# deu439/ARFlow

Hardware: AMD Instinct MI355X
Metric: image-pairs/sec fwd+bwd, PWCLite 384x640 bs=8 (higher is better)
Workload: dtype f32; 1 GPU; pwclite_uflow+uflow_loss, 384x640 pairs, batch 8 per GPU, fwd(both directions)+loss+bwd+allreduce+Adam; global_batch=8, parallelism=dp1, step_start=seeded weights + fresh Adam state, restored before every step, loss_finite=True

## Files before the change

### arflow_amd/_lib.py

```python
import ctypes
import os

_HERE = os.path.dirname(os.path.abspath(__file__))
LIB_PATH = os.path.join(_HERE, 'csrc', 'libarflow_hip.so')

c_fp = ctypes.c_void_p
c_i = ctypes.c_int
c_l = ctypes.c_long
c_f = ctypes.c_float

PROTOTYPES = {
    'arflow_abi_version': [],
    'arflow_take_stale_error': [],
    'arflow_set_deterministic': [c_i],
    'arflow_get_deterministic': [],
    'arflow_flow_up_fwd': [c_fp, c_fp, c_i, c_i, c_i, c_i, c_i, c_fp],
    'arflow_flow_up_bwd': [c_fp, c_fp, c_i, c_i, c_i, c_i, c_i, c_fp],
    'arflow_out_up2_fwd': [c_fp, c_l, c_fp, c_l, c_i, c_i, c_i, c_i, c_i, c_i, c_f, c_fp],
    'arflow_out_up2_bwd': [c_fp, c_l, c_fp, c_l, c_i, c_i, c_i, c_i, c_i, c_fp],
    'arflow_out_tail_fwd': [c_fp, c_l, c_fp, c_fp, c_i, c_i, c_i, c_i, c_i, c_i, c_f, c_fp],
    'arflow_prob_up_fwd': [c_fp, c_l, c_fp, c_l, c_i, c_i, c_i, c_i, c_i, c_i, c_i, c_f, c_fp],
    'arflow_prob_up_bwd': [c_fp, c_l, c_fp, c_l, c_i, c_i, c_i, c_i, c_i, c_i, c_fp],
    'arflow_profile_marker': [c_i, c_fp],
    'arflow_sums_rows': [c_i, c_i, c_i],
    'arflow_corr_fwd': [c_fp, c_fp, c_fp, c_fp, c_i, c_i, c_i, c_i, c_i, c_f, c_fp],
    'arflow_corr_sign_planes': [c_i, c_i, c_i],
    'arflow_corr_strided_supported': [c_i, c_i, c_i],
    'arflow_corr_fwd_strided': [c_fp, c_fp, c_fp, c_l, c_fp, c_i, c_i, c_i, c_i, c_i, c_f, c_fp],
    'arflow_corr_bwd_strided': [c_fp, c_l, c_fp, c_l, c_fp, c_fp, c_fp, c_fp, c_fp, c_i, c_i, c_i, c_i, c_i, c_f, c_fp],
    'arflow_corr_bwd': [c_fp, c_fp, c_fp, c_fp, c_fp, c_fp, c_fp, c_i, c_i, c_i, c_i, c_i, c_f, c_fp],
    'arflow_corr_fwd_bf16': [c_fp, c_fp, c_fp, c_i, c_i, c_i, c_i, c_i, c_f, c_fp],
    'arflow_corr_bwd_bf16': [c_fp, c_fp, c_fp, c_fp, c_fp, c_fp, c_i, c_i, c_i, c_i, c_i, c_f, c_fp],
    'arflow_warp_fwd_bf16': [c_fp, c_fp, c_fp, c_fp, c_i, c_i, c_i, c_i, c_i, c_i, c_l, c_i, c_i, c_i, c_fp],
    'arflow_warp_bwd_bf16': [c_fp, c_fp, c_fp, c_fp, c_fp, c_i, c_i, c_i, c_i, c_i, c_i, c_l, c_i, c_i, c_i, c_fp],
    'arflow_warp_nearest_fwd': [c_fp, c_fp, c_fp, c_i, c_i, c_i, c_i, c_i, c_i, c_l, c_i, c_i, c_i, c_fp],
    'arflow_warp_nearest_bwd': [c_fp, c_fp, c_fp, c_i, c_i, c_i, c_i, c_i, c_i, c_l, c_i, c_i, c_i, c_fp],
    'arflow_warp_bicubic_fwd': [c_fp, c_fp, c_fp, c_i, c_i, c_i, c_i, c_i, c_i, c_l, c_i, c_i, c_i, c_fp],
    'arflow_warp_bicubic_bwd': [c_fp, c_fp, c_fp, c_fp, c_fp, c_i, c_i, c_i, c_i, c_i, c_i, c_l, c_i, c_i, c_i, c_fp],
    'arflow_ssim_fwd': [c_fp, c_fp, c_fp, c_i, c_i, c_i, c_i, c_i, c_fp],
    'arflow_ssim_bwd': [c_fp, c_fp, c_fp, c_fp, c_i, c_i, c_i, c_i, c_i, c_fp],
    'arflow_corr_general_out_size': [c_i, c_i, c_i, c_i, c_i, c_i, c_i, c_fp, c_fp, c_fp],
    'arflow_corr_general_fwd': [c_fp, c_fp, c_fp, c_i, c_i, c_i, c_i, c_i, c_i, c_i, c_i, c_i, c_fp],
    'arflow_corr_general_bwd': [c_fp, c_fp, c_fp, c_fp, c_fp, c_i, c_i, c_i, c_i, c_i, c_i, c_i, c_i, c_i, c_fp],
    'arflow_featnorm_fwd': [c_fp, c_fp, c_fp, c_fp, c_fp, c_fp, c_i, c_l, c_i, c_fp],
    'arflow_featnorm_bwd': [c_fp, c_fp, c_fp, c_fp, c_fp, c_fp, c_fp, c_fp, c_i, c_l, c_i, c_fp],
    'arflow_level_supported': [c_i, c_i, c_i],
    'arflow_level_bwd_ws_bytes': [c_i, c_i, c_i, c_i],
    'arflow_level_fwd': [c_fp, c_fp, c_fp, c_l, c_i, c_i, c_fp, c_fp, c_l, c_fp, c_i, c_fp, c_l, c_fp, c_l, c_fp, c_fp, c_fp, c_i, c_i, c_i, c_i, c_i, c_f, c_i, c_i, c_i, c_fp],
    'arflow_level_bwd': [c_fp, c_l, c_fp, c_fp, c_l, c_fp, c_l, c_fp, c_fp, c_fp, c_fp, c_l, c_fp, c_l, c_fp, c_fp, c_i, c_fp, c_fp, c_fp, c_i, c_i, c_fp, c_i, c_i, c_i, c_i, c_i, c_f, c_i, c_i, c_i, c_fp],
    'arflow_level_fwd_m': [c_fp, c_fp, c_fp, c_l, c_i, c_i, c_fp, c_fp, c_l, c_fp, c_i, c_fp, c_l, c_fp, c_l, c_fp, c_fp, c_fp, c_fp, c_i, c_fp, c_i, c_i, c_i, c_i, c_i, c_i, c_f, c_i, c_i, c_i, c_fp],
    'arflow_up2_bwd': [c_fp, c_fp, c_i, c_i, c_i, c_i, c_fp],
    'arflow_bias_act_mom_rows': [c_i, c_l],
    'arflow_bias_act_fwd_mom': [c_fp, c_fp, c_fp, c_fp, c_i, c_i, c_l, c_f, c_fp],
    'arflow_level_acc_rows': [c_i, c_i, c_i, c_i, c_i],
    'arflow_level_moments': [c_fp, c_fp, c_fp, c_i, c_l, c_fp],
    'arflow_level_warp_fwd': [c_fp, c_fp, c_fp, c_l, c_i, c_i, c_fp, c_fp, c_l, c_fp, c_fp, c_i, c_i, c_i, c_i, c_i, c_i, c_i, c_fp],
    'arflow_level_corr_fwd': [c_fp, c_fp, c_fp, c_i, c_i, c_fp, c_l, c_fp, c_l, c_fp, c_fp, c_i, c_i, c_i, c_i, c_i, c_f, c_fp],
    'arflow_level_corr_bwd': [c_fp, c_l, c_fp, c_fp, c_l, c_fp, c_fp, c_fp, c_fp, c_i, c_i, c_i, c_i, c_i, c_f, c_fp],
    'arflow_bias_act_fwd': [c_fp, c_fp, c_fp, c_i, c_i, c_l, c_f, c_fp],
    'arflow_bias_act_bwd': [c_fp, c_fp, c_fp, c_fp, c_i, c_i, c_l, c_f, c_fp],
    'arflow_headconv_fwd': [c_fp, c_fp, c_fp, c_fp, c_i, c_i, c_i, c_i, c_fp],
    'arflow_headconv_bwd_data': [c_fp, c_fp, c_fp, c_i, c_i, c_i, c_i, c_fp],
    'arflow_headconv_bwd_weight_ws_bytes': [c_i, c_i, c_i, c_i],
    'arflow_headconv_bwd_weight': [c_fp, c_fp, c_fp, c_fp, c_fp, c_i, c_i, c_i, c_i, c_fp],
    'arflow_splitconv_pack_bytes': [c_i, c_i],
    'arflow_splitconv_pack': [c_fp, c_fp, c_i, c_i, c_i, c_fp],
    'arflow_splitconv_fwd': [c_fp, c_fp, c_fp, c_i, c_i, c_i, c_i, c_i, c_fp],
    'arflow_dense_cat_fwd': [c_fp, c_fp, c_fp, c_fp, c_i, c_i, c_i, c_l, c_f, c_fp],
    'arflow_dense_gbias_rows': [c_i, c_l],
    'arflow_dense_grad_gather': [c_fp, c_i, c_fp, c_l, c_fp, c_fp, c_i, c_i, c_l, c_f, c_fp],
    'arflow_warp_fwd': [c_fp, c_fp, c_fp, c_fp, c_i, c_i, c_i, c_i, c_i, c_i, c_l, c_i, c_i, c_i, c_fp],
    'arflow_warp_bwd': [c_fp, c_fp, c_fp, c_fp, c_fp, c_i, c_i, c_i, c_i, c_i, c_i, c_l, c_i, c_i, c_i, c_fp],
    'arflow_splat_map': [c_fp, c_fp, c_i, c_i, c_i, c_l, c_i, c_fp],
    'arflow_coord_mask': [c_fp, c_fp, c_i, c_i, c_i, c_l, c_i, c_fp],
    'arflow_occ_bidir': [c_fp, c_fp, c_fp, c_i, c_i, c_i, c_l, c_l, c_f, c_f, c_fp],
    'arflow_census_fwd': [c_fp, c_fp, c_fp, c_fp, c_fp, c_fp, c_i, c_i, c_i, c_i, c_fp],
    'arflow_census_bwd': [c_fp, c_fp, c_fp, c_fp, c_fp, c_i, c_i, c_i, c_i, c_fp],
    'arflow_census_warp_supported': [c_i, c_i],
    'arflow_census_warp_fwd': [c_fp, c_fp, c_fp, c_l, c_fp, c_fp, c_fp, c_fp, c_i, c_i, c_i, c_i, c_fp],
    'arflow_census_warp_bwd': [c_fp, c_fp, c_fp, c_l, c_fp, c_fp, c_fp, c_i, c_i, c_i, c_i, c_fp],
    'arflow_census_warp_pair_fwd': [c_fp, c_fp, c_l, c_fp, c_fp, c_fp, c_fp, c_i, c_i, c_i, c_i, c_fp],
    'arflow_census_warp_pair_bwd': [c_fp, c_fp, c_l, c_fp, c_fp, c_fp, c_i, c_i, c_i, c_i, c_fp],
    'arflow_uflow_pair_bwd': [c_fp, c_fp, c_l, c_fp, c_fp, c_fp, c_i, c_i, c_i, c_i, c_fp, c_l, c_fp, c_fp, c_fp, c_i, c_i, c_f, c_f, c_i, c_i, c_i, c_fp],
    'arflow_down4_gray_z': [c_fp, c_fp, c_fp, c_fp, c_i, c_i, c_i, c_fp],
    'arflow_splat_smooth_fwd': [c_fp, c_fp, c_fp, c_fp, c_i, c_i, c_i, c_l, c_f, c_f, c_i, c_i, c_i, c_i, c_fp],
    'arflow_down4_gray': [c_fp, c_fp, c_fp, c_i, c_i, c_i, c_fp],
    'arflow_photo_fwd': [c_fp, c_fp, c_fp, c_fp, c_fp, c_i, c_i, c_i, c_i, c_fp],
    'arflow_photo_bwd': [c_fp, c_fp, c_fp, c_fp, c_fp, c_fp, c_i, c_i, c_i, c_i, c_fp],
    'arflow_photo_warp_rows': [c_i, c_i, c_i],
    'arflow_photo_warp_fwd': [c_fp, c_l, c_l, c_fp, c_l, c_l, c_fp, c_l, c_l, c_fp, c_l, c_l, c_i, c_i, c_i, c_i, c_fp, c_fp, c_i, c_i, c_i, c_i, c_i, c_i, c_fp],
    'arflow_photo_warp_bwd': [c_fp, c_l, c_l, c_fp, c_l, c_l, c_fp, c_l, c_l, c_fp, c_l, c_l, c_i, c_i, c_i, c_i, c_fp, c_fp, c_l, c_l, c_i, c_i, c_i, c_i, c_i, c_i, c_fp],
    'arflow_area_pyramid_ws_bytes': [c_i, c_i, c_i, c_fp, c_i],
    'arflow_area_pyramid': [c_fp, c_fp, c_i, c_i, c_i, c_fp, c_i, c_fp],
    'arflow_smooth_fwd': [c_fp, c_fp, c_fp, c_i, c_i, c_i, c_i, c_l, c_f, c_f, c_i, c_i, c_i, c_fp],
    'arflow_smooth_bwd': [c_fp, c_fp, c_fp, c_fp, c_i, c_i, c_i, c_i, c_l, c_f, c_f, c_i, c_i, c_i, c_fp],
    'arflow_down4': [c_fp, c_fp, c_i, c_i, c_i, c_fp],
    'arflow_up4_clamp_mul': [c_fp, c_fp, c_fp, c_i, c_i, c_i, c_fp],
    'arflow_flow_eval_rows': [c_i, c_i],
    'arflow_flow_eval': [c_fp, c_fp, c_fp, c_fp, c_fp, c_i, c_i, c_i, c_i, c_i, c_i, c_fp],
    'arflow_triag_solve': [c_fp, c_fp, c_fp, c_fp, c_fp, c_fp, c_i, c_i, c_i, c_i, c_fp],
    'arflow_triag_solve_bwd': [c_fp, c_fp, c_fp, c_fp, c_fp, c_fp, c_fp, c_fp, c_fp, c_fp, c_fp, c_i, c_i, c_i, c_i, c_fp],
    'arflow_triag_inverse_diagonal': [c_fp, c_fp, c_fp, c_fp, c_i, c_i, c_i, c_fp],
    'arflow_band_mv_fwd': [c_fp, c_l, c_fp, c_l, c_fp, c_l, c_fp, c_l, c_fp, c_l, c_i, c_i, c_i, c_i, c_i, c_i, c_fp],
    'arflow_band_mv_bwd': [c_fp, c_l, c_fp, c_l, c_fp, c_l, c_fp, c_l, c_fp, c_l, c_fp, c_l, c_fp, c_l, c_fp, c_l, c_i, c_i, c_i, c_i, c_i, c_i, c_fp],
    'arflow_lowrank_sample_fwd': [c_fp, c_l, c_fp, c_l, c_fp, c_fp, c_l, c_i, c_i, c_i, c_i, c_i, c_fp],
    'arflow_lowrank_work_size': [c_i, c_i, c_i, c_i],
    'arflow_lowrank_logdet_fwd': [c_fp, c_l, c_fp, c_fp, c_fp, c_i, c_i, c_i, c_i, c_fp],
    'arflow_lowrank_bwd': [c_fp, c_l, c_fp, c_fp, c_l, c_fp, c_fp, c_fp, c_l, c_fp, c_l, c_i, c_i, c_i, c_i, c_i, c_fp],
    'arflow_mixture_work_size': [c_i, c_i, c_i, c_i, c_i],
    'arflow_mixture_sample_fwd': [c_fp, c_l, c_fp, c_l, c_fp, c_l, c_fp, c_fp, c_l, c_fp, c_i, c_i, c_i, c_i, c_i, c_fp],
    'arflow_mixture_logpdf_fwd': [c_fp, c_fp, c_fp, c_fp, c_fp, c_i, c_i, c_i, c_i, c_i, c_fp],
    'arflow_mixture_bwd': [c_fp, c_l, c_fp, c_l, c_fp, c_l, c_fp, c_fp, c_fp, c_fp, c_l, c_fp, c_l, c_fp, c_l, c_i, c_i, c_i, c_i, c_i, c_fp],
    'arflow_mixture_entropy_map': [c_fp, c_l, c_fp, c_l, c_fp, c_fp, c_fp, c_l, c_fp, c_i, c_i, c_i, c_i, c_i, c_fp],
    'arflow_gauss_pyr_work_size': [c_fp, c_fp, c_i, c_i],
    'arflow_gauss_pyr_sample_fwd': [c_fp, c_fp, c_fp, c_fp, c_fp, c_fp, c_fp, c_fp, c_i, c_i, c_fp, c_fp, c_fp],
    'arflow_gauss_pyr_sample_bwd': [c_fp, c_fp, c_fp, c_fp, c_fp, c_fp, c_fp, c_fp, c_fp, c_fp, c_fp, c_i, c_i, c_fp],
    'arflow_mse_work_size': [c_i, c_i, c_i],
    'arflow_mse_fwd': [c_fp, c_l, c_i, c_fp, c_l, c_i, c_i, c_fp, c_l, c_i, c_i, c_i, c_i, c_i, c_i, c_fp, c_fp, c_fp],
    'arflow_mse_bwd': [c_fp, c_l, c_i, c_fp, c_l, c_i, c_i, c_fp, c_l, c_fp, c_fp, c_l, c_fp, c_l, c_i, c_i, c_i, c_i, c_i, c_i, c_fp],
    'arflow_resize_flow': [c_fp, c_l, c_i, c_i, c_fp, c_l, c_i, c_i, c_i, c_i, c_fp],
# ... 50 lines not shown
```

### arflow_amd/functional.py

```python
import contextlib

import torch

from . import _lib
from . import ddp as _ddp

PAD = {'zeros': 0, 'border': 1}
NORM_ARFLOW, NORM_UFLOW = 0, 1


def _need_gpu(*tensors):
    for t in tensors:
        if t is None:
            continue
        if not t.is_cuda:
            raise _lib.ArflowHipError('arflow_amd ops run on the GPU only (got a %s tensor); there is no CPU '
                                      'fallback -- the CPU oracle lives in oracle/ and is test-only' % t.device)
        if t.dtype != torch.float32:
            raise _lib.ArflowHipError('arflow_amd ops are fp32 only (got %s)' % t.dtype)


def _p(t):
    return None if t is None else t.data_ptr()

# ... 567 lines not shown
                    dw = None
        return dx, dw, db


def head_conv(x, weight, bias):
    return HeadConvFunction.apply(x, weight, bias)


def head_conv_enabled():
    return _HEADCONV


_SPLITCONV = __import__('os').environ.get('ARFLOW_SPLITCONV', '1') != '0'


def splitconv_enabled():
    return _SPLITCONV


def splitconv_takes(N, C, K, H, W):
    if not _SPLITCONV:
        return False
    return _splitconv_rule(int(N), int(C), int(K), int(H), int(W))


def _splitconv_rule(N, C, K, H, W):
    if min(C, K) < 32 or not 64 <= max(C, K) <= 640:
        return False
    if H * W >= 96 * 160 and N * H * W >= 16 * 96 * 160:
        return True
    if H * W >= 48 * 80 and N * H * W >= 16 * 48 * 80:
        return max(C, K) >= 128 and (K >= 128 or C <= 128)
    return False


def splitconv(x, w, transpose_flip=False):
    _need_gpu(x, w)
    if x.dim() != 4 or w.dim() != 4 or tuple(w.shape[2:]) != (3, 3) or x.shape[1] != w.shape[0 if transpose_flip else 1]:
        raise ValueError('splitconv expects x [N,C,H,W] and w [K,C,3,3] (transpose_flip: x [N,K,H,W])')
    x, w = x.contiguous(), w.contiguous()
    N, C, H, W = x.shape
    K = int(w.shape[1 if transpose_flip else 0])
    nbytes = _lib.load().arflow_splitconv_pack_bytes(K, C)
    if nbytes < 0:
        _lib.check(int(nbytes), 'arflow_splitconv_pack_bytes')
    packed = torch.empty(nbytes, device=x.device, dtype=torch.uint8)
    y = torch.empty(N, K, H, W, device=x.device, dtype=torch.float32)
    with torch.cuda.device_of(x):
        _call('arflow_splitconv_pack', _p(w), _p(packed), int(w.shape[0]), int(w.shape[1]), int(bool(transpose_flip)), _stream())
        _call('arflow_splitconv_fwd', _p(x), _p(packed), _p(y), N, C, K, H, W, _stream())
    return y


def _conv_args():
    return [1, 1], [1, 1], [1, 1], False, [0, 0], 1


class Conv3x3Function(torch.autograd.Function):

    @staticmethod
    def forward(ctx, x, w, fwd, dgrad):
        if fwd:
            y = splitconv(x, w)
        else:
            y = torch.ops.aten.convolution(x, w, None, *_conv_args())
        ctx.save_for_backward(x, w)
        ctx.dgrad = bool(dgrad)
        return y

    @staticmethod
    @torch.autograd.function.once_differentiable
    def backward(ctx, gy):
        x, w = ctx.saved_tensors
        gy = gy.contiguous()
        want_dx, want_dw = ctx.needs_input_grad[0], ctx.needs_input_grad[1]
        dx = dw = None
        if ctx.dgrad and want_dx:
            dx = splitconv(gy, w, transpose_flip=True)
            want_dx = False
        if want_dx or want_dw:
            dx_m, dw, _ = torch.ops.aten.convolution_backward(gy, x, w, None, *_conv_args(), [want_dx, want_dw, False])
            if want_dx:
                dx = dx_m
            if not want_dw:
                dw = None
        return dx, dw, None, None


def conv3x3(x, w, fwd=True, dgrad=True):
    return Conv3x3Function.apply(x, w, bool(fwd), bool(dgrad))


_DENSE_BLOCK = __import__('os').environ.get('ARFLOW_DENSE_BLOCK', '1') != '0'
DENSE_MAX_SRC = 8


def dense_block_enabled():
    return _DENSE_BLOCK


def _dense_src_type():
    import ctypes

    class DenseSrc(ctypes.Structure):
        _fields_ = [('ptr', ctypes.c_void_p), ('bstride', ctypes.c_long), ('scale', ctypes.c_void_p)]
    return DenseSrc


_DenseSrc = _dense_src_type()


def dense_cat(y, bias, x, slope):
    _need_gpu(y, bias, x)
    if y.dim() != 4 or x.dim() != 4 or y.shape[0] != x.shape[0] or y.shape[2:] != x.shape[2:]:
        raise ValueError('dense_cat expects y [B,oc,H,W] and x [B,C,H,W]')
    y, x = y.contiguous(), x.contiguous()
    bias = None if bias is None else bias.contiguous()
    B, oc, H, W = y.shape
    C = x.shape[1]
    out = torch.empty(B, oc + C, H, W, device=y.device, dtype=torch.float32)
    with torch.cuda.device_of(y):
        _call('arflow_dense_cat_fwd', _p(y), _p(bias), _p(x), _p(out), B, oc, C, H * W, float(slope), _stream(),
              key=(B, oc, C, H * W))
    return out


def dense_grad_gather(sources, oc, act=None, slope=0.1, want_bias=False):
    import ctypes
    if not 1 <= len(sources) <= DENSE_MAX_SRC:
        raise ValueError('dense_grad_gather takes 1..%d sources' % DENSE_MAX_SRC)
    t0 = sources[0][0]
    B, _, H, W = t0.shape
    hw = H * W
    arr = (_DenseSrc * len(sources))()
    keep = []
    for j, (t, off, scale) in enumerate(sources):
        _need_gpu(t, scale)
        st = t.stride()
        if t.dim() != 4 or t.shape[0] != B or tuple(t.shape[2:]) != (H, W) or off < 0 or off + oc > t.shape[1]:
            raise ValueError('dense_grad_gather: source %d does not hold channels %d:%d of a [%d,*,%d,%d] tensor' % (j, off, off + oc, B, H, W))
        if st[3] != 1 or st[2] != W or st[1] != hw:
            t = t.contiguous()
            st = t.stride()
# ... 41 lines not shown
                y = splitconv(xk, w)
            else:
                y = torch.nn.functional.conv2d(xk, w, None, 1, 1)
            xs.append(dense_cat(y, b, xk, slope))
        x6 = xs[-1]
        B, C6, H, W = x6.shape
        w_head = w_head.contiguous()
        flow = torch.empty(B, 2, H, W, device=x.device, dtype=torch.float32)
        with torch.cuda.device_of(x6):
            _call('arflow_headconv_fwd', _p(x6), _p(w_head), _p(b_head.contiguous()), _p(flow), B, C6, H, W, _stream())
        ctx.save_for_backward(*xs, *ws, w_head)
        ctx.slope = slope
        ctx.set_materialize_grads(False)
        return x6, flow

    @staticmethod
    @torch.autograd.function.once_differentiable
    def backward(ctx, gx6, gflow):
        xs, ws, w_head = ctx.saved_tensors[:6], ctx.saved_tensors[6:11], ctx.saved_tensors[11]
        need = ctx.needs_input_grad
        grads = [None] * 14
        if gx6 is None and gflow is None:
            return tuple(grads)
        x6 = xs[5]
        B, C6, H, W = x6.shape
        ocs = [int(w.shape[0]) for w in ws]
        lowest = 0 if need[0] else next((m for m in range(1, 6) if need[2 * m] or need[2 * m + 1]), 6)
        dx_head = None
        with torch.cuda.device_of(x6):
            if gflow is not None:
                gflow = gflow.contiguous()
                if lowest < 6:
                    dx_head = torch.empty_like(x6)
                    _call('arflow_headconv_bwd_data', _p(gflow), _p(w_head), _p(dx_head), B, C6, H, W, _stream())
                if need[12] or need[13]:
                    nbytes = _lib.load().arflow_headconv_bwd_weight_ws_bytes(B, C6, H, W)
                    if nbytes < 0:
                        _lib.check(int(nbytes), 'arflow_headconv_bwd_weight_ws_bytes')
                    wsb = torch.empty(nbytes, device=x6.device, dtype=torch.uint8)
                    dw = torch.empty_like(w_head)
                    db = torch.empty(2, device=x6.device, dtype=torch.float32) if need[13] else None
                    _call('arflow_headconv_bwd_weight', _p(x6), _p(gflow), _p(dw), _p(db), _p(wsb), B, C6, H, W, _stream())
                    grads[12], grads[13] = (dw if need[12] else None), db
        if lowest == 6:
            return tuple(grads)
        top = [t for t in (gx6, dx_head) if t is not None]
        dxs = []
        for m in range(5, max(lowest, 1) - 1, -1):
            srcs = [(t, sum(ocs[m:5]), None) for t in top] + [(dx, sum(ocs[m:k - 1]), None) for dx, k in dxs]
            gy, gb = dense_grad_gather(srcs, ocs[m - 1], act=xs[m], slope=ctx.slope, want_bias=need[2 * m + 1])
            want_dx = m > lowest
            dx = dw = None
            xm = xs[m - 1]
            if want_dx and splitconv_takes(B, ocs[m - 1], xm.shape[1], H, W):
                dx = splitconv(gy, ws[m - 1], transpose_flip=True)
                if need[2 * m]:
                    dw = torch.ops.aten.convolution_backward(gy, xm, ws[m - 1], None, *_conv_args(), [False, True, False])[1]
            elif want_dx or need[2 * m]:
                dx, dw, _ = torch.ops.aten.convolution_backward(gy, xm, ws[m - 1], None, *_conv_args(),
                                                                [want_dx, bool(need[2 * m]), False])
            grads[2 * m], grads[2 * m + 1] = (dw if need[2 * m] else None), gb
            if want_dx:
                dxs.append((dx, m))
        if need[0]:
            srcs = [(t, sum(ocs), None) for t in top] + [(dx, sum(ocs[:k - 1]), None) for dx, k in dxs]
            grads[0] = dense_grad_gather(srcs, int(xs[0].shape[1]))[0]
        return tuple(grads)


def dense_estimator(x, slope, params):
    return DenseEstimatorFunction.apply(x, slope, *params)


@_samples_mode
class BiasLeakyReLUMomentsFunction(torch.autograd.Function):

    @staticmethod
    def forward(ctx, x, bias, slope):
        _need_gpu(x)
        if not x.is_contiguous():
            raise ValueError('bias_leaky_relu expects a contiguous [B,C,...] tensor')
        B, C = x.shape[0], x.shape[1]
        hw = x[0, 0].numel()
        if bias is not None:
            _need_gpu(bias)
            bias = bias.contiguous()
        rows = _lib.load().arflow_bias_act_mom_rows(C, hw)
        mom = torch.empty(B, rows, 2, device=x.device, dtype=torch.float64)
        with torch.cuda.device_of(x):
            _call('arflow_bias_act_fwd_mom', _p(x), _p(bias), _p(x), _p(mom), B, C, hw, float(slope), _stream(), key=(B, C, hw))
        ctx.mark_dirty(x)
        ctx.mark_non_differentiable(mom)
        ctx.save_for_backward(x)
        ctx.slope, ctx.has_bias = float(slope), bias is not None
        return x, mom

    @staticmethod
    def backward(ctx, gout, gmom_unused):
        y, = ctx.saved_tensors
        B, C = y.shape[0], y.shape[1]
        hw = y[0, 0].numel()
        gout = gout.contiguous()
        gin = torch.empty_like(gout)
        gb = torch.empty(C, device=y.device, dtype=torch.float32) if (ctx.has_bias and ctx.needs_input_grad[1]) else None
        with torch.cuda.device_of(y):
            _call('arflow_bias_act_bwd', _p(gout), _p(y), _p(gin), _p(gb), B, C, hw, ctx.slope, _stream(), key=(B, C, hw))
        return gin, gb, None


def bias_leaky_relu_moments(x, bias, slope=0.1):
    return BiasLeakyReLUMomentsFunction.apply(x, bias, slope)


# ... 1089 lines not shown
```

### arflow_amd/models/blocks.py

```python
import torch
import torch.nn as nn
import torch.nn.functional as F

from .. import functional as AF

bias_act = AF.bias_leaky_relu


class ConvAct(nn.Sequential):

    want_moments = False
    last_moments = None

    def split_route(self, x):
        c = self[0]
        if not (AF.splitconv_enabled() and bias_act is AF.bias_leaky_relu and x.is_cuda and x.dtype == torch.float32 and
                x.dim() == 4 and c.weight.dtype == torch.float32 and c.kernel_size == (3, 3) and c.stride == (1, 1) and
                c.padding == (1, 1) and c.dilation == (1, 1) and c.groups == 1 and c.padding_mode == 'zeros'):
            return False, False
        N, C, H, W = x.shape
        return AF.splitconv_takes(N, C, c.out_channels, H, W), AF.splitconv_takes(N, c.out_channels, C, H, W)

    def forward(self, x):
        c, act = self[0], self[1]
        fwd, dgrad = self.split_route(x)
        if fwd or dgrad:
            y = AF.conv3x3(x, c.weight, fwd, dgrad)
        else:
            y = F.conv2d(x, c.weight, None, c.stride, c.padding, c.dilation, c.groups)
        if self.want_moments and y.is_cuda and bias_act is AF.bias_leaky_relu:
            y, self.last_moments = AF.bias_leaky_relu_moments(y, c.bias, act.negative_slope)
            return y
        self.last_moments = None
        return bias_act(y, c.bias, act.negative_slope)


class HeadConv(nn.Sequential):

    def native(self, x):
        c = self[0]
        return (AF.head_conv_enabled() and bias_act is AF.bias_leaky_relu and x.is_cuda and x.dtype == torch.float32 and
                x.dim() == 4 and c.weight.dtype == torch.float32 and c.out_channels == 2 and c.kernel_size == (3, 3) and
                c.stride == (1, 1) and c.padding == (1, 1) and c.dilation == (1, 1) and c.groups == 1 and
                c.padding_mode == 'zeros')

    def forward(self, x):
        c = self[0]
        if self.native(x):
            return AF.head_conv(x, c.weight, c.bias)
        return F.conv2d(x, c.weight, c.bias, c.stride, c.padding, c.dilation, c.groups)


def conv(in_planes, out_planes, kernel_size=3, stride=1, dilation=1, isReLU=True):
    layers = [nn.Conv2d(in_planes, out_planes, kernel_size=kernel_size, stride=stride, dilation=dilation,
                        padding=((kernel_size - 1) * dilation) // 2, bias=True)]
    if isReLU:
        layers.append(nn.LeakyReLU(0.1, inplace=True))
        return ConvAct(*layers)
    return HeadConv(*layers)


def deconv(in_planes, out_planes, kernel_size=4, stride=2, padding=1):
    return nn.ConvTranspose2d(in_planes, out_planes, kernel_size, stride, padding, bias=True)


class FeatureExtractor(nn.Module):

    def __init__(self, num_chs, convs_per_level=2, rescale_input=False, moments=False):
        super().__init__()
        self.num_chs = num_chs
        self.rescale_input = rescale_input
        self.convs = nn.ModuleList()
        for ch_in, ch_out in zip(num_chs[:-1], num_chs[1:]):
            layers = [conv(ch_in, ch_out, stride=2)] + [conv(ch_out, ch_out) for _ in range(convs_per_level - 1)]
            layers[-1].want_moments = bool(moments)
            self.convs.append(nn.Sequential(*layers))
        self.pyramid_moments = None

    def forward(self, x):
        if self.rescale_input:
# ... 98 lines not shown
```

### include/arflow_hip.h

```cpp
#ifndef ARFLOW_HIP_H
#define ARFLOW_HIP_H

#ifdef __cplusplus
extern "C" {
#endif

typedef void* arflow_stream_t;

#define ARFLOW_OK 0
#define ARFLOW_ENULL (-1001)
#define ARFLOW_ESHAPE (-1002)
#define ARFLOW_EPARAM (-1003)
#define ARFLOW_ENONDET (-1004)
#define ARFLOW_ELAUNCH_BASE (-2000)

#define ARFLOW_PAD_ZEROS 0
#define ARFLOW_PAD_BORDER 1

#define ARFLOW_NORM_ARFLOW 0
#define ARFLOW_NORM_UFLOW 1
#define ARFLOW_NORM_UFLOW_ABS 2
#define ARFLOW_COORDS_ABS 2

#define ARFLOW_SUM_COLS 4
// ... 49 lines not shown
int arflow_level_supported(int C, int W, int max_disp);
long arflow_level_bwd_ws_bytes(int B, int C, int H, int W);
int arflow_level_fwd(const float* x1, const float* x2, const float* flow, long flow_bstride, int flow_is_coarse,
                     int up_align_corners, float* flow_up, float* flow_up2, long flow_up2_bstride, float* x2w, int norm_mode,
                     float* out, long out_bstride, float* x1n, long x1n_bstride, unsigned* sign_bits, float* stats,
                     double* acc, int B, int C, int H, int W, int max_disp, float negative_slope, int pad_mode,
                     int align_corners, int coord_norm, arflow_stream_t stream);
int arflow_level_fwd_m(const float* x1, const float* x2, const float* flow, long flow_bstride, int flow_is_coarse,
                       int up_align_corners, float* flow_up, float* flow_up2, long flow_up2_bstride, float* x2w, int norm_mode,
                       float* out, long out_bstride, float* x1n, long x1n_bstride, unsigned* sign_bits, float* stats,
                       double* acc, const double* x1_rows, int x1_nrows, const double* x2_rows, int x2_nrows, int B, int C, int H,
                       int W, int max_disp, float negative_slope, int pad_mode, int align_corners, int coord_norm,
                       arflow_stream_t stream);
int arflow_level_bwd(const float* gout, long gout_bstride, const unsigned* sign_bits, const float* x1n, long x1n_bstride,
                     const float* gx1n_direct, long gx1n_direct_bstride, const float* x1, const float* x2, const float* x2w,
                     const float* flow_full, long flow_bstride, const float* gflow_a, long gflow_a_bstride,
                     const float* gflow_b, const float* stats, int norm_mode, float* gx1, float* gx2, float* gflow,
                     int flow_is_coarse, int up_align_corners, void* workspace, int B, int C, int H, int W, int max_disp,
                     float negative_slope, int pad_mode, int align_corners, int coord_norm, arflow_stream_t stream);
int arflow_level_acc_rows(int B, int C, int H, int W, int has_flow);
int arflow_up2_bwd(const float* gfine, float* gcoarse, int B, int H, int W, int up_align_corners, arflow_stream_t stream);
int arflow_level_moments(const float* x1, const float* x2, double* acc, int B, long n, arflow_stream_t stream);
int arflow_level_warp_fwd(const float* x1, const float* x2, const float* flow, long flow_bstride, int flow_is_coarse,
                          int up_align_corners, float* flow_up, float* flow_up2, long flow_up2_bstride, float* x2w,
                          double* acc, int B, int C, int H, int W, int pad_mode, int align_corners, int norm_mode,
                          arflow_stream_t stream);
int arflow_level_corr_fwd(const float* x1, const float* x2w, const double* acc, int acc_rows, int norm_mode, float* out,
                          long out_bstride, float* x1n, long x1n_bstride, unsigned* sign_bits, float* stats, int B, int C,
                          int H, int W, int max_disp, float negative_slope, arflow_stream_t stream);
int arflow_level_corr_bwd(const float* gout, long gout_bstride, const unsigned* sign_bits, const float* x1n,
                          long x1n_bstride, const float* x2w, const float* stats, float* gx1n, float* gx2n, int B, int C,
                          int H, int W, int max_disp, float negative_slope, arflow_stream_t stream);

int arflow_bias_act_fwd(const float* x, const float* bias, float* y, int B, int C, long HW,
                        float negative_slope, arflow_stream_t stream);
int arflow_bias_act_mom_rows(int C, long HW);
int arflow_bias_act_fwd_mom(const float* x, const float* bias, float* y, double* mom, int B, int C, long HW,
                            float negative_slope, arflow_stream_t stream);
int arflow_bias_act_bwd(const float* gout, const float* y, float* gin, float* gbias, int B, int C, long HW,
                        float negative_slope, arflow_stream_t stream);

int arflow_headconv_fwd(const float* x, const float* w, const float* bias, float* y, int B, int C, int H, int W,
                        arflow_stream_t stream);
int arflow_headconv_bwd_data(const float* dy, const float* w, float* dx, int B, int C, int H, int W,
                             arflow_stream_t stream);
long arflow_headconv_bwd_weight_ws_bytes(int B, int C, int H, int W);
int arflow_headconv_bwd_weight(const float* x, const float* dy, float* dw, float* dbias, void* ws, int B, int C, int H,
                               int W, arflow_stream_t stream);

long arflow_splitconv_pack_bytes(int K, int C);
int arflow_splitconv_pack(const float* w, void* packed, int K, int C, int transpose_flip, arflow_stream_t stream);
int arflow_splitconv_fwd(const float* x, const void* packed, float* y, int N, int C, int K, int H, int W,
                         arflow_stream_t stream);

#define ARFLOW_DENSE_MAX_SRC 8
typedef struct {
  const float* ptr;
  long bstride;
  const float* scale;
} arflow_dense_src;
int arflow_dense_cat_fwd(const float* y, const float* bias, const float* x, float* out, int B, int oc, int C, long HW,
                         float negative_slope, arflow_stream_t stream);
int arflow_dense_gbias_rows(int B, long HW);
int arflow_dense_grad_gather(const arflow_dense_src* srcs, int n_src, const float* act, long act_bs, float* gy,
                             float* gbias_rows, int B, int oc, long HW, float negative_slope, arflow_stream_t stream);

int arflow_warp_fwd(const float* src, const float* flow, float* out, float* valid, int B, int C,
                    int Hs, int Ws, int H, int W, long flow_bstride, int pad_mode, int align_corners,
                    int norm_mode, arflow_stream_t stream);

int arflow_warp_bwd(const float* gout, const float* src, const float* flow, float* gsrc, float* gflow,
                    int B, int C, int Hs, int Ws, int H, int W, long flow_bstride, int pad_mode,
                    int align_corners, int norm_mode, arflow_stream_t stream);

int arflow_splat_map(const float* flow, float* out, int B, int H, int W, long flow_bstride,
                     int variant, arflow_stream_t stream);

int arflow_coord_mask(const float* flow, float* out, int B, int H, int W, long flow_bstride, int mode,
                      arflow_stream_t stream);

int arflow_occ_bidir(const float* flow12, const float* flow21, float* out, int B, int H, int W,
                     long bstride12, long bstride21, float scale, float bias, arflow_stream_t stream);

int arflow_census_fwd(const float* im_a, const float* im_b, const float* mask, float* ham, float* dham,
                      float* sums, int B, int H, int W, int radius, arflow_stream_t stream);

int arflow_census_bwd(const float* im_a, const float* im_b, const float* gham, const float* scale,
                      float* g_im_b, int B, int H, int W, int radius, arflow_stream_t stream);

int arflow_census_warp_supported(int H, int W);
int arflow_census_warp_fwd(const float* gray_a, const float* gray_b, const float* flow, long flow_bstride,
                           const float* occ_small, float* mask_out, float* dham, float* sums, int B, int H, int W,
                           int radius, arflow_stream_t stream);
int arflow_census_warp_bwd(const float* gray_a, const float* gray_b, const float* flow, long flow_bstride,
                           const float* dham, const float* scale, float* gflow, int B, int H, int W, int radius,
                           arflow_stream_t stream);
int arflow_census_warp_pair_fwd(const float* gray, const float* flow, long flow_bstride, const float* occ_small,
                                float* mask_out, float* dham, float* sums, int B2, int H, int W, int radius,
                                arflow_stream_t stream);
int arflow_census_warp_pair_bwd(const float* gray, const float* flow, long flow_bstride, const float* dham,
                                const float* scale2, float* gflow, int B2, int H, int W, int radius, arflow_stream_t stream);
int arflow_uflow_pair_bwd(const float* gray, const float* flow, long flow_bstride, const float* dham, const float* scale2,
                          float* gflow, int B2, int H, int W, int radius, const float* flow2, long flow2_bstride,
                          const float* img2, const float* coef2, float* gflow2, int h2, int w2, float flow_scale, float alpha,
                          int order, int wmode, int penalty, arflow_stream_t stream);
int arflow_down4_gray(const float* im, float* small, float* gray, int B, int H, int W, arflow_stream_t stream);
// ... 155 lines not shown
```

Measured before the change: 169.2 image-pairs/s.

## Add split-bf16 MFMA weight-gradient kernel for large 3x3 convs

Adds a HIP kernel that computes the 3x3 conv weight gradient with bf16 MFMA 32x32x16 instructions. It splits fp32 values three ways into bf16 parts to keep near-fp32 accuracy, and reduces per-chunk partials into a workspace finished in double precision. The kernel is routed in for the dense-block and conv-block backward when the shape rule matches (C 448-640, K 32-128, large spatial), replacing aten convolution_backward for dw. The cost is a workspace allocation plus a separate reduction pass, and the path only fires for a narrow set of shapes.

```diff
diff --git a/arflow_amd/_lib.py b/arflow_amd/_lib.py
--- a/arflow_amd/_lib.py
+++ b/arflow_amd/_lib.py
@@ -66,6 +66,8 @@
     'arflow_splitconv_pack_bytes': [c_i, c_i],
     'arflow_splitconv_pack': [c_fp, c_fp, c_i, c_i, c_i, c_fp],
     'arflow_splitconv_fwd': [c_fp, c_fp, c_fp, c_i, c_i, c_i, c_i, c_i, c_fp],
+    'arflow_splitconv_wgrad_ws_bytes': [c_i, c_i, c_i, c_i, c_i],
+    'arflow_splitconv_wgrad': [c_fp, c_l, c_fp, c_l, c_fp, c_fp, c_i, c_i, c_i, c_i, c_i, c_fp],
     'arflow_dense_cat_fwd': [c_fp, c_fp, c_fp, c_fp, c_i, c_i, c_i, c_l, c_f, c_fp],
     'arflow_dense_gbias_rows': [c_i, c_l],
     'arflow_dense_grad_gather': [c_fp, c_i, c_fp, c_l, c_fp, c_fp, c_i, c_i, c_l, c_f, c_fp],
diff --git a/arflow_amd/csrc/splitconv_wgrad.hip b/arflow_amd/csrc/splitconv_wgrad.hip
--- /dev/null
+++ b/arflow_amd/csrc/splitconv_wgrad.hip
@@ -0,0 +1,315 @@
+#include <climits>
+#include <cstdint>
+
+#include "common.hpp"
+
+namespace {
+typedef __bf16 bf16x8 __attribute__((ext_vector_type(8)));
+typedef float f32x16 __attribute__((ext_vector_type(16)));
+typedef unsigned u32x4 __attribute__((ext_vector_type(4)));
+
+constexpr int G = 8;
+constexpr int DY_CS = 3 * G + 1;
+constexpr int X_CS = 9 * G + 1;
+constexpr int XH_CS = 9 * G + 1;
+constexpr int MAX_ROWS = 128;
+constexpr int MIN_ROWS = 4;
+constexpr int WANT_WG = 1024;
+constexpr int MAX_KT = 2;
+
+template <int KT>
+struct Lds {
+  static constexpr int DY = 0;
+  static constexpr int X = KT * 32 * DY_CS * 16;
+  static constexpr int XH = X + 32 * X_CS * 16;
+  static constexpr int BYTES = XH + 32 * XH_CS * 4;
+};
+
+struct Split {
+  __bf16 p[3];
+  __device__ __forceinline__ explicit Split(float v) {
+    p[0] = (__bf16)v;
+    const float r1 = v - (float)p[0];
+    p[1] = (__bf16)r1;
+    p[2] = (__bf16)(r1 - (float)p[1]);
+  }
+};
+__device__ __forceinline__ unsigned bf16_bits(__bf16 b) { return (unsigned)__builtin_bit_cast(unsigned short, b); }
+
+struct Run {
+  float4 a, b;
+  float l, r;
+};
+template <bool VEC>
+__device__ __forceinline__ void load_run(const float* __restrict__ row, int col0, int W, bool valid, Run& o) {
+  const float4 z = make_float4(0.f, 0.f, 0.f, 0.f);
+  if (VEC) {
+    const bool in0 = col0 < W, in1 = col0 + 4 < W;
+    const float4 t0 = *reinterpret_cast<const float4*>(row + (in0 ? col0 : 0));
+    const float4 t1 = *reinterpret_cast<const float4*>(row + (in1 ? col0 + 4 : 0));
+    o.a = valid && in0 ? t0 : z;
+    o.b = valid && in1 ? t1 : z;
+  } else {
+    float t[8];
+#pragma unroll
+    for (int e = 0; e < 8; ++e) t[e] = row[min(col0 + e, W - 1)];
+#pragma unroll
+    for (int e = 0; e < 8; ++e) t[e] = (valid && col0 + e < W) ? t[e] : 0.f;
+    o.a = make_float4(t[0], t[1], t[2], t[3]);
+    o.b = make_float4(t[4], t[5], t[6], t[7]);
+  }
+}
+
+struct Plan {
+  int GW, SG, nstrips, RPC, nrb, nct, nkt, kchunks;
+  long chunks;
+};
+inline int tiles32(int n) { return (n + 31) / 32; }
+inline bool shape_ok(int N, int C, int K, int H, int W) {
+  return N > 0 && C > 0 && K > 0 && H > 0 && W > 0 && (long)N * C * H * W <= INT_MAX && (long)N * K * H * W <= INT_MAX &&
+         (long)9 * K * C <= INT_MAX;
+}
+inline Plan make_plan(int N, int C, int K, int H, int W) {
+  Plan p;
+  p.GW = (W + 7) / 8;
+  const int ns = (p.GW + G - 1) / G;
+  p.SG = 2 * ((p.GW + 2 * ns - 1) / (2 * ns));
+  p.nstrips = (p.GW + p.SG - 1) / p.SG;
+  p.nct = tiles32(C), p.nkt = tiles32(K), p.kchunks = (p.nkt + MAX_KT - 1) / MAX_KT;
+  const long units = (long)p.nct * p.kchunks * N * p.nstrips;
+  const long want = (WANT_WG + units - 1) / units;
+  int rpc = (int)((H + want - 1) / want);
+  if (rpc < MIN_ROWS) rpc = MIN_ROWS;
+  if (rpc > MAX_ROWS) rpc = MAX_ROWS;
+  if (rpc > H) rpc = H;
+  p.RPC = rpc;
+  p.nrb = (H + rpc - 1) / rpc;
+  p.chunks = (long)N * p.nstrips * p.nrb;
+  return p;
+}
+
+template <int KT, bool VEC>
+__global__ __launch_bounds__(192 * KT, VEC && KT == 2 ? 3 : 2) void splitconv_wgrad_kernel(const float* __restrict__ x, long x_bs,
+                                                                             const float* __restrict__ dy, long dy_bs,
+                                                                             float* __restrict__ ws, int C, int K, int H, int W,
+                                                                             int kt_first, int kcnt, int nct, int nstrips, int SG,
+                                                                             int nrb, int RPC) {
+  constexpr int NT = 192 * KT;
+  using L = Lds<KT>;
+  extern __shared__ __align__(16) unsigned char lds[];
+  unsigned* const xh = reinterpret_cast<unsigned*>(lds + L::XH);
+  const int tid = threadIdx.x, lane = tid & 63, wv = __builtin_amdgcn_readfirstlane(tid >> 6);
+  const int r32 = lane & 31, hh = lane >> 5;
+  const int ktl = wv / 3, tr = wv - 3 * ktl;
+  const int b = blockIdx.x;
+  const int ct = b % nct, kc = (b / nct) % kcnt, chunk = b / (nct * kcnt);
+  const int rb = chunk % nrb, strip = (chunk / nrb) % nstrips, n = chunk / (nrb * nstrips);
+  const int kt0 = kt_first + kc * KT;
+  const int h0 = rb * RPC, h1 = min(H, h0 + RPC);
+  const int GW = (W + 7) >> 3, g0 = strip * SG, gcount = min(SG, GW - g0), nsteps = (gcount + 1) >> 1;
+  const long HWl = (long)H * W;
+  const float* const xn = x + (long)n * x_bs;
+  const float* const dyn = dy + (long)n * dy_bs;
+
+  constexpr int NX = 32 * G, NITEM = NX + KT * 32 * G, NSLOT = (NITEM + NT - 1) / NT;
+  Run pf[NSLOT];
+  const auto fetch = [&](int yx, int ydy) __attribute__((always_inline)) {
+#pragma unroll
+    for (int j = 0; j < NSLOT; ++j) {
+      const int i = tid + j * NT;
+      if (i < NX) {
+        const int cl = i / G, g = i - cl * G;
+        const int c = ct * 32 + cl, col0 = (g0 + g) * 8;
+        const bool valid = yx >= 0 && yx < H && c < C && g < gcount;
+        const float* row = xn + (valid ? (long)c * HWl + (long)yx * W : 0);
+        load_run<VEC>(row, col0, W, valid, pf[j]);
+        const float vl = row[max(col0 - 1, 0)], vr = row[min(col0 + 8, W - 1)];
+        pf[j].l = (valid && col0 > 0) ? vl : 0.f;
+        pf[j].r = (valid && col0 + 8 < W) ? vr : 0.f;
+      } else if (i < NITEM && ydy >= 0) {
+        const int kl = (i - NX) / G, g = (i - NX) - kl * G;
+        const int k = kt0 * 32 + kl, col0 = (g0 + g) * 8;
+        const bool valid = k < K && g < gcount;
+        const float* row = dyn + (valid ? (long)k * HWl + (long)ydy * W : 0);
+        load_run<VEC>(row, col0, W, valid, pf[j]);
+      }
+    }
+  };
+  const auto commit = [&](int yx, int ydy) __attribute__((always_inline)) {
+    const int slot = (yx + 3) % 3;
+#pragma unroll
+    for (int j = 0; j < NSLOT; ++j) {
+      const int i = tid + j * NT;
+      if (i < NX) {
+        const int cl = i / G, g = i - cl * G;
+        const float v[8] = {pf[j].a.x, pf[j].a.y, pf[j].a.z, pf[j].a.w, pf[j].b.x, pf[j].b.y, pf[j].b.z, pf[j].b.w};
+        bf16x8 o[3];
+#pragma unroll
+        for (int e = 0; e < 8; ++e) {
+          const Split s(v[e]);
+          o[0][e] = s.p[0], o[1][e] = s.p[1], o[2][e] = s.p[2];
+        }
+        const Split sl(pf[j].l), sr(pf[j].r);
+#pragma unroll
+        for (int p = 0; p < 3; ++p) {
+          const int at = (slot * 3 + p) * G + g;
+          *reinterpret_cast<bf16x8*>(lds + L::X + (cl * X_CS + at) * 16) = o[p];
+          xh[cl * XH_CS + at] = (bf16_bits(sl.p[p]) << 16) | bf16_bits(sr.p[p]);
+        }
+      } else if (i < NITEM && ydy >= 0) {
+        const int kl = (i - NX) / G, g = (i - NX) - kl * G;
+        const float v[8] = {pf[j].a.x, pf[j].a.y, pf[j].a.z, pf[j].a.w, pf[j].b.x, pf[j].b.y, pf[j].b.z, pf[j].b.w};
+        bf16x8 o[3];
+#pragma unroll
+        for (int e = 0; e < 8; ++e) {
+          const Split s(v[e]);
+          o[0][e] = s.p[0], o[1][e] = s.p[1], o[2][e] = s.p[2];
+        }
+#pragma unroll
+        for (int p = 0; p < 3; ++p) *reinterpret_cast<bf16x8*>(lds + L::DY + (kl * DY_CS + p * G + g) * 16) = o[p];
+      }
+    }
+  };
+
+  f32x16 tot[3];
+#pragma unroll
+  for (int s = 0; s < 3; ++s)
+#pragma unroll
+    for (int i = 0; i < 16; ++i) tot[s][i] = 0.f;
+
+  const unsigned char* const a_base = lds + L::DY + ((ktl * 32 + r32) * DY_CS + hh) * 16;
+  fetch(h0 - 1, -1);
+  commit(h0 - 1, -1);
+  fetch(h0, -1);
+  commit(h0, -1);
+  fetch(h0 + 1, h0);
+  for (int h = h0; h < h1; ++h) {
+    if (h > h0) __syncthreads();
+    commit(h + 1, h);
+    __syncthreads();
+    fetch(h + 2, h + 1 < h1 ? h + 1 : -1);
+    const int slot = (h + tr + 2) % 3;
+    const unsigned char* const b_base = lds + L::X + (r32 * X_CS + slot * 3 * G + hh) * 16;
+    const unsigned* const bh_base = xh + r32 * XH_CS + slot * 3 * G + hh;
+    f32x16 acc[3];
+#pragma unroll
+    for (int s = 0; s < 3; ++s)
+#pragma unroll
+      for (int i = 0; i < 16; ++i) acc[s][i] = 0.f;
+    const auto x_frags = [&](int p, int t, bf16x8 (&bs)[3]) __attribute__((always_inline)) {
+      const u32x4 d = *reinterpret_cast<const u32x4*>(b_base + (p * G + 2 * t) * 16);
+      const unsigned nb = bh_base[p * G + 2 * t];
+      const unsigned m1 = __builtin_amdgcn_alignbit(d.y, d.x, 16), m2 = __builtin_amdgcn_alignbit(d.z, d.y, 16),
+                     m3 = __builtin_amdgcn_alignbit(d.w, d.z, 16);
+      const u32x4 lo = {__builtin_amdgcn_alignbit(d.x, nb, 16), m1, m2, m3};
+      const u32x4 hi = {m1, m2, m3, __builtin_amdgcn_alignbit(nb, d.w, 16)};
+      bs[0] = __builtin_bit_cast(bf16x8, lo);
+      bs[1] = __builtin_bit_cast(bf16x8, d);
+      bs[2] = __builtin_bit_cast(bf16x8, hi);
+    };
+#pragma unroll 1
+    for (int t = 0; t < nsteps; ++t) {
+      bf16x8 a[3], bs[3];
+#pragma unroll
+      for (int p = 0; p < 3; ++p) a[p] = *reinterpret_cast<const bf16x8*>(a_base + (p * G + 2 * t) * 16);
+#pragma unroll
+      for (int p = 2; p >= 0; --p) {
+        x_frags(p, t, bs);
+#pragma unroll
+        for (int pa = 2 - p; pa >= (p == 0 ? 1 : 0); --pa)
+#pragma unroll
+          for (int s = 0; s < 3; ++s) acc[s] = __builtin_amdgcn_mfma_f32_32x32x16_bf16(a[pa], bs[s], acc[s], 0, 0, 0);
+      }
+    }
+#pragma unroll 1
+    for (int t = 0; t < nsteps; ++t) {
+      bf16x8 bs[3];
+      const bf16x8 a0 = *reinterpret_cast<const bf16x8*>(a_base + (2 * t) * 16);
+      x_frags(0, t, bs);
+#pragma unroll
+      for (int s = 0; s < 3; ++s) acc[s] = __builtin_amdgcn_mfma_f32_32x32x16_bf16(a0, bs[s], acc[s], 0, 0, 0);
+    }
+#pragma unroll
+    for (int s = 0; s < 3; ++s) tot[s] = tot[s] + acc[s];
+  }
+  const int c = ct * 32 + r32;
+  if (c < C) {
+#pragma unroll
+    for (int s = 0; s < 3; ++s) {
+      float* const wt = ws + ((long)chunk * 9 + (tr * 3 + s)) * K * C;
+#pragma unroll
+      for (int i = 0; i < 16; ++i) {
+        const int k = 32 * (kt0 + ktl) + (i & 3) + 8 * (i >> 2) + 4 * hh;
+        if (k < K) wt[(long)k * C + c] = tot[s][i];
+      }
+    }
+  }
+}
+
+__global__ __launch_bounds__(256) void splitconv_wgrad_finish_kernel(const float* __restrict__ ws, float* __restrict__ dw, int K,
+                                                                       int C, int chunks) {
+  const int KC = K * C, e = blockIdx.x * 256 + threadIdx.x;
+  if (e >= 9 * KC) return;
+  const int tap = e / KC, kc = e - tap * KC;
+  double s = 0.0;
+  for (int ch = 0; ch < chunks; ++ch) s += (double)ws[(long)ch * 9 * KC + e];
+  dw[(long)kc * 9 + tap] = (float)s;
+}
+
+template <int KT, bool VEC>
+int launch(const float* x, long x_bs, const float* dy, long dy_bs, float* ws, int C, int K, int H, int W, int kt_first, int kcnt,
+           const Plan& p, hipStream_t st) {
+  using L = Lds<KT>;
+  static bool attr_set = false;
+  if (!attr_set) {
+    const hipError_t e = hipFuncSetAttribute(reinterpret_cast<const void*>(&splitconv_wgrad_kernel<KT, VEC>),
+                                             hipFuncAttributeMaxDynamicSharedMemorySize, L::BYTES);
+    if (e != hipSuccess) return af_hip_status(e);
+    attr_set = true;
+  }
+  const long grid = p.chunks * kcnt * p.nct;
+  if (grid > INT_MAX) return ARFLOW_ESHAPE;
+  hipLaunchKernelGGL((splitconv_wgrad_kernel<KT, VEC>), dim3((unsigned)grid), dim3(192 * KT), L::BYTES, st, x, x_bs, dy, dy_bs, ws, C, K,
+                     H, W, kt_first, kcnt, p.nct, p.nstrips, p.SG, p.nrb, p.RPC);
+  return af_launch_status();
+}
+}
+
+extern "C" long arflow_splitconv_wgrad_ws_bytes(int N, int C, int K, int H, int W) {
+  if (!shape_ok(N, C, K, H, W)) return ARFLOW_ESHAPE;
+  const Plan p = make_plan(N, C, K, H, W);
+  if (p.chunks > INT_MAX) return ARFLOW_ESHAPE;
+  return p.chunks * 9 * K * C * 4;
+}
+
+extern "C" int arflow_splitconv_wgrad(const float* x, long x_bstride, const float* dy, long dy_bstride, float* dw, void* ws, int N,
+                                      int C, int K, int H, int W, arflow_stream_t stream) {
+  af_clear_stale_error();
+  AF_REQUIRE_PTR(x);
+  AF_REQUIRE_PTR(dy);
+  AF_REQUIRE_PTR(dw);
+  AF_REQUIRE_PTR(ws);
+  AF_REQUIRE(shape_ok(N, C, K, H, W), ARFLOW_ESHAPE);
+  AF_REQUIRE(af_stride_ok(x_bstride, N, (long)C * H * W) && af_stride_ok(dy_bstride, N, (long)K * H * W), ARFLOW_ESHAPE);
+  AF_REQUIRE(x_bstride >= 0 && dy_bstride >= 0 && x_bstride <= LONG_MAX / N && dy_bstride <= LONG_MAX / N, ARFLOW_ESHAPE);
+  AF_REQUIRE((((uintptr_t)x | (uintptr_t)dy | (uintptr_t)dw) & 3) == 0 && af_aligned16(ws), ARFLOW_EPARAM);
+  const Plan p = make_plan(N, C, K, H, W);
+  AF_REQUIRE(p.chunks <= INT_MAX, ARFLOW_ESHAPE);
+  hipStream_t st = (hipStream_t)stream;
+  const bool vec = W % 4 == 0 && af_vec4_ok(x, x_bstride, N) && af_vec4_ok(dy, dy_bstride, N);
+  const int base = p.nkt / p.kchunks, extra = p.nkt % p.kchunks;
+  for (int part = 0; part < 2; ++part) {
+    const int kt = part == 0 ? base + 1 : base, cnt = part == 0 ? extra : p.kchunks - extra, first = part == 0 ? 0 : extra * (base + 1);
+    if (cnt == 0) continue;
+    const auto go = [&](auto kt_c, auto vec_c) {
+      return launch<decltype(kt_c)::value, decltype(vec_c)::value>(x, x_bstride, dy, dy_bstride, (float*)ws, C, K, H, W, first, cnt, p, st);
+    };
+    using std::integral_constant;
+    const int rc = kt == 1 ? (vec ? go(integral_constant<int, 1>{}, std::true_type{}) : go(integral_constant<int, 1>{}, std::false_type{}))
+                           : (vec ? go(integral_constant<int, 2>{}, std::true_type{}) : go(integral_constant<int, 2>{}, std::false_type{}));
+    if (rc != ARFLOW_OK) return rc;
+  }
+  hipLaunchKernelGGL(splitconv_wgrad_finish_kernel, dim3((unsigned)af_cdiv((long)9 * K * C, 256)), dim3(256), 0, st,
+                     (const float*)ws, dw, K, C, (int)p.chunks);
+  return af_launch_status();
+}
diff --git a/arflow_amd/functional.py b/arflow_amd/functional.py
--- a/arflow_amd/functional.py
+++ b/arflow_amd/functional.py
@@ -643,6 +643,46 @@
     return y
 
 
+_SPLITCONV_WGRAD = __import__('os').environ.get('ARFLOW_SPLITCONV_WGRAD', '1') != '0'
+
+
+def splitconv_wgrad_takes(N, C, K, H, W):
+    if not (_SPLITCONV and _SPLITCONV_WGRAD):
+        return False
+    return _splitconv_wgrad_rule(int(N), int(C), int(K), int(H), int(W))
+
+
+def _splitconv_wgrad_rule(N, C, K, H, W):
+    if N * H * W < 16 * 48 * 80:
+        return False
+    return H * W >= 96 * 160 and N * H * W >= 16 * 96 * 160 and 448 <= C <= 640 and 32 <= K <= 128
+
+
+def _batch_strided(t):
+    _, C, H, W = t.shape
+    if t.stride(3) != 1 or t.stride(2) != W or t.stride(1) != H * W or (t.shape[0] > 1 and t.stride(0) < C * H * W):
+        t = t.contiguous()
+    return t, (int(t.stride(0)) if t.shape[0] > 1 else C * H * W)
+
+
+def splitconv_wgrad(x, gy):
+    _need_gpu(x, gy)
+    if x.dim() != 4 or gy.dim() != 4 or x.shape[0] != gy.shape[0] or x.shape[2:] != gy.shape[2:]:
+        raise ValueError('splitconv_wgrad expects x [N,C,H,W] and gy [N,K,H,W]')
+    x, x_bs = _batch_strided(x)
+    gy, gy_bs = _batch_strided(gy)
+    N, C, H, W = x.shape
+    K = int(gy.shape[1])
+    nbytes = _lib.load().arflow_splitconv_wgrad_ws_bytes(N, C, K, H, W)
+    if nbytes < 0:
+        _lib.check(int(nbytes), 'arflow_splitconv_wgrad_ws_bytes')
+    ws = torch.empty(nbytes, device=x.device, dtype=torch.uint8)
+    dw = torch.empty(K, C, 3, 3, device=x.device, dtype=torch.float32)
+    with torch.cuda.device_of(x):
+        _call('arflow_splitconv_wgrad', _p(x), x_bs, _p(gy), gy_bs, _p(dw), _p(ws), N, C, K, H, W, _stream())
+    return dw
+
+
 def _conv_args():
     return [1, 1], [1, 1], [1, 1], False, [0, 0], 1
 
@@ -650,13 +690,13 @@
 class Conv3x3Function(torch.autograd.Function):
 
     @staticmethod
-    def forward(ctx, x, w, fwd, dgrad):
+    def forward(ctx, x, w, fwd, dgrad, wgrad=False):
         if fwd:
             y = splitconv(x, w)
         else:
             y = torch.ops.aten.convolution(x, w, None, *_conv_args())
         ctx.save_for_backward(x, w)
-        ctx.dgrad = bool(dgrad)
+        ctx.dgrad, ctx.wgrad = bool(dgrad), bool(wgrad)
         return y
 
     @staticmethod
@@ -669,17 +709,20 @@
         if ctx.dgrad and want_dx:
             dx = splitconv(gy, w, transpose_flip=True)
             want_dx = False
+        if ctx.wgrad and want_dw:
+            dw = splitconv_wgrad(x, gy)
+            want_dw = False
         if want_dx or want_dw:
-            dx_m, dw, _ = torch.ops.aten.convolution_backward(gy, x, w, None, *_conv_args(), [want_dx, want_dw, False])
+            dx_m, dw_m, _ = torch.ops.aten.convolution_backward(gy, x, w, None, *_conv_args(), [want_dx, want_dw, False])
             if want_dx:
                 dx = dx_m
-            if not want_dw:
-                dw = None
-        return dx, dw, None, None
-
-
-def conv3x3(x, w, fwd=True, dgrad=True):
-    return Conv3x3Function.apply(x, w, bool(fwd), bool(dgrad))
+            if want_dw:
+                dw = dw_m
+        return dx, dw, None, None, None
+
+
+def conv3x3(x, w, fwd=True, dgrad=True, wgrad=False):
+    return Conv3x3Function.apply(x, w, bool(fwd), bool(dgrad), bool(wgrad))
 
 
 _DENSE_BLOCK = __import__('os').environ.get('ARFLOW_DENSE_BLOCK', '1') != '0'
@@ -827,13 +870,19 @@
             want_dx = m > lowest
             dx = dw = None
             xm = xs[m - 1]
-            if want_dx and splitconv_takes(B, ocs[m - 1], xm.shape[1], H, W):
+            ask_dx, ask_dw = want_dx, bool(need[2 * m])
+            if ask_dx and splitconv_takes(B, ocs[m - 1], xm.shape[1], H, W):
                 dx = splitconv(gy, ws[m - 1], transpose_flip=True)
-                if need[2 * m]:
-                    dw = torch.ops.aten.convolution_backward(gy, xm, ws[m - 1], None, *_conv_args(), [False, True, False])[1]
-            elif want_dx or need[2 * m]:
-                dx, dw, _ = torch.ops.aten.convolution_backward(gy, xm, ws[m - 1], None, *_conv_args(),
-                                                                [want_dx, bool(need[2 * m]), False])
+                ask_dx = False
+            if ask_dw and splitconv_wgrad_takes(B, xm.shape[1], ocs[m - 1], H, W):
+                dw = splitconv_wgrad(xm, gy)
+                ask_dw = False
+            if ask_dx or ask_dw:
+                dx_m, dw_m, _ = torch.ops.aten.convolution_backward(gy, xm, ws[m - 1], None, *_conv_args(), [ask_dx, ask_dw, False])
+                if ask_dx:
+                    dx = dx_m
+                if ask_dw:
+                    dw = dw_m
             grads[2 * m], grads[2 * m + 1] = (dw if need[2 * m] else None), gb
             if want_dx:
                 dxs.append((dx, m))
diff --git a/arflow_amd/models/blocks.py b/arflow_amd/models/blocks.py
--- a/arflow_amd/models/blocks.py
+++ b/arflow_amd/models/blocks.py
@@ -13,19 +13,30 @@
     last_moments = None
 
     def split_route(self, x):
+        if not self._split_kind(x):
+            return False, False
         c = self[0]
-        if not (AF.splitconv_enabled() and bias_act is AF.bias_leaky_relu and x.is_cuda and x.dtype == torch.float32 and
-                x.dim() == 4 and c.weight.dtype == torch.float32 and c.kernel_size == (3, 3) and c.stride == (1, 1) and
-                c.padding == (1, 1) and c.dilation == (1, 1) and c.groups == 1 and c.padding_mode == 'zeros'):
-            return False, False
         N, C, H, W = x.shape
         return AF.splitconv_takes(N, C, c.out_channels, H, W), AF.splitconv_takes(N, c.out_channels, C, H, W)
+
+    def split_wgrad_route(self, x):
+        if not self._split_kind(x):
+            return False
+        N, C, H, W = x.shape
+        return AF.splitconv_wgrad_takes(N, C, self[0].out_channels, H, W)
+
+    def _split_kind(self, x):
+        c = self[0]
+        return (AF.splitconv_enabled() and bias_act is AF.bias_leaky_relu and x.is_cuda and x.dtype == torch.float32 and
+                x.dim() == 4 and c.weight.dtype == torch.float32 and c.kernel_size == (3, 3) and c.stride == (1, 1) and
+                c.padding == (1, 1) and c.dilation == (1, 1) and c.groups == 1 and c.padding_mode == 'zeros')
 
     def forward(self, x):
         c, act = self[0], self[1]
         fwd, dgrad = self.split_route(x)
-        if fwd or dgrad:
-            y = AF.conv3x3(x, c.weight, fwd, dgrad)
+        wgrad = self.split_wgrad_route(x)
+        if fwd or dgrad or wgrad:
+            y = AF.conv3x3(x, c.weight, fwd, dgrad, wgrad)
         else:
             y = F.conv2d(x, c.weight, None, c.stride, c.padding, c.dilation, c.groups)
         if self.want_moments and y.is_cuda and bias_act is AF.bias_leaky_relu:
diff --git a/include/arflow_hip.h b/include/arflow_hip.h
--- a/include/arflow_hip.h
+++ b/include/arflow_hip.h
@@ -125,6 +125,10 @@
 int arflow_splitconv_pack(const float* w, void* packed, int K, int C, int transpose_flip, arflow_stream_t stream);
 int arflow_splitconv_fwd(const float* x, const void* packed, float* y, int N, int C, int K, int H, int W,
                          arflow_stream_t stream);
+
+long arflow_splitconv_wgrad_ws_bytes(int N, int C, int K, int H, int W);
+int arflow_splitconv_wgrad(const float* x, long x_bstride, const float* dy, long dy_bstride, float* dw, void* ws, int N, int C,
+                           int K, int H, int W, arflow_stream_t stream);
 
 #define ARFLOW_DENSE_MAX_SRC 8
 typedef struct {
```

New measurement: 171.5 image-pairs/s (median of 6 runs). 1.01x the previous value.
